# JackWoo0831/Yolov7-tracker

Measured on AMD Instinct MI355X. Metric: end-to-end fps (detect+track) YOLOv7-w6@1280 ByteTrack, higher is better.
Workload: dtype f16

## Files before the change

yolov7-tracker_amd/csrc/y7t_conv_ws_s2.hip:

```cpp
#include "y7t_common.h"
#include "y7t_conv_common.h"
#include <stdlib.h>

namespace {

#if defined(Y7T_CONVSIM)
#define WS2_VMCNT(dev, dma) cs_vmcnt(dma)
#else
#define WS2_VMCNT(dev, dma) asm volatile("s_waitcnt vmcnt(" #dev ")" ::: "memory")
#endif

struct Ws2 {
    static constexpr int TW = 32, TH = 2;
    static constexpr int PIXB = 144;
    static constexpr int NE = TW + 1, NO = TW;
    static constexpr int O_OFF = NE * PIXB;
    static constexpr int RP = (NE + NO) * PIXB;
    static constexpr int ROWS = 2 * TH + 1;
    static constexpr int PATCH_DMA = (ROWS * RP + 1023) / 1024;
    static constexpr int PATCH_BYTES = PATCH_DMA * 1024;
    static constexpr int NPW = (PATCH_DMA + 3) / 4;
    static constexpr int NBUF = 3;
    static constexpr int OUT_OFF = NBUF * PATCH_BYTES;
    static constexpr int LDS = OUT_OFF + TW * TH * 256;
    static constexpr int NSUB = 36;
    static constexpr unsigned OOB = 0xFF000000u;
};

template <int ACT, bool FUSE>
__global__ void __launch_bounds__(256, 1) k_conv3x3s2_c64_ws(const Y7TConvArgs p) {
#if defined(__HIP_DEVICE_COMPILE__)
    using C = Ws2;
    constexpr int TW = C::TW, TH = C::TH, PIXB = C::PIXB, RP = C::RP, NPW = C::NPW;
    extern __shared__ __attribute__((aligned(16))) char smem[];
    const int tid = threadIdx.x, lane = tid & 63, wave = __builtin_amdgcn_readfirstlane(tid >> 6);
    const int l31 = lane & 31, hi32 = lane >> 5;

    const int tiles_x = p.Wo / TW, tiles_y = p.Ho / TH, ptiles = p.B * tiles_y * tiles_x;
    int bid = blockIdx.x;
    if (p.xcd_swizzle) {
        const int nwg = gridDim.x, q = nwg >> 3, r = nwg & 7, xcd = bid & 7, idx = bid >> 3;
        bid = (xcd < r ? xcd * (q + 1) : r * (q + 1) + (xcd - r) * q) + idx;
    }
    const int per = (ptiles + (int)gridDim.x - 1) / (int)gridDim.x;
    const int pt_first = bid * per;
    const int nt = (ptiles - pt_first) < per ? (ptiles - pt_first) : per;
    if (nt <= 0) return;

    const __amdgpu_buffer_rsrc_t xr = __builtin_amdgcn_make_buffer_rsrc((void*)p.in, 0, p.in_bytes, 0x00020000);

    struct TileIt { int b, ty, tx, n; };
    auto tile_it = [&](int pt) -> TileIt {
        int q = pt;
        const int txi = q % tiles_x; q /= tiles_x;
        return TileIt{q / tiles_y, q % tiles_y, txi, pt_first + nt - pt};
    };
    auto tile_next = [&](TileIt& it) __attribute__((always_inline)) {
        it.n -= 1;
        if (++it.tx == tiles_x) { it.tx = 0; if (++it.ty == tiles_y) { it.ty = 0; ++it.b; } }
    };
    unsigned pconst[NPW], pedge = 0;
#pragma unroll
    for (int i = 0; i < NPW; ++i) {
        int I = wave + 4 * i;
        if (I >= C::PATCH_DMA) I = C::PATCH_DMA - 1;
        const int byte = I * 1024 + lane * 16;
        const int r = byte / RP, rb = byte - r * RP;
        const int px = rb / PIXB, cs = (rb - px * PIXB) >> 4;
        const int pc = px < C::NE ? 2 * px : 2 * (px - C::NE) + 1;
        const bool used = r < C::ROWS && cs < 8;
        pconst[i] = used ? (unsigned)(((r * p.W + pc) * p.ldin + cs * 8) * 2) : 0u;
        const unsigned e = used ? (unsigned)((r == 0) | ((pc == 0) << 1)) : 0u;
        pedge |= e << (2 * i);
    }
    auto piece_offsets = [&](const TileIt& it, unsigned (&pv)[NPW]) __attribute__((always_inline)) {
        const unsigned org = ((((unsigned)it.b * (unsigned)p.H + (unsigned)(2 * it.ty * TH) - 1u) * (unsigned)p.W + (unsigned)(2 * it.tx * TW) - 1u) * (unsigned)p.ldin +
                              (unsigned)p.cin_off) * 2u;
        const unsigned tmask = (unsigned)((it.ty == 0) | ((it.tx == 0) << 1));
#pragma unroll
        for (int i = 0; i < NPW; ++i) pv[i] = (it.n <= 0 || ((pedge >> (2 * i)) & tmask)) ? C::OOB : pconst[i] + org;
    };
    auto issue_piece = [&](int buf, unsigned v, int i) __attribute__((always_inline)) {
        const int I = (wave + 4 * i < C::PATCH_DMA) ? wave + 4 * i : C::PATCH_DMA - 1;
        __builtin_amdgcn_raw_ptr_buffer_load_lds(xr, (LDS_AS void*)(smem + buf * C::PATCH_BYTES + I * 1024), 16, v, 0, 0, 0);
    };

    half8 wreg[C::NSUB];
    {
        const half8* wp = (const half8*)p.w + wave * 64 + lane;
#pragma unroll
        for (int f = 0; f < C::NSUB; ++f) wreg[f] = wp[f * 256];
    }
    floatx16 biasv;
#pragma unroll
    for (int g = 0; g < 4; ++g)
#pragma unroll
        for (int e = 0; e < 4; ++e) biasv[g * 4 + e] = p.bias[wave * 32 + 8 * g + 4 * hi32 + e];

    half8 w2reg[FUSE ? 8 : 1];
    floatx16 bias2v;
    if (FUSE) {
        const half8* wp2 = (const half8*)p.w + C::NSUB * 256 + wave * 64 + lane;
#pragma unroll
        for (int ks = 0; ks < 8; ++ks) w2reg[ks] = wp2[ks * 256];
#pragma unroll
        for (int g = 0; g < 4; ++g)
#pragma unroll
            for (int e = 0; e < 4; ++e) bias2v[g * 4 + e] = p.bias[128 + wave * 32 + 8 * g + 4 * hi32 + e];
    }

    unsigned pv[NPW];
    TileIt itn = tile_it(pt_first), ito = itn;
    piece_offsets(itn, pv);
#pragma unroll
    for (int i = 0; i < NPW; ++i) issue_piece(0, pv[i], i);
    tile_next(itn);
    piece_offsets(itn, pv);
#pragma unroll
    for (int i = 0; i < NPW; ++i) issue_piece(1, pv[i], i);
    tile_next(itn);

    const int plane_off = l31 * PIXB + hi32 * 16;
    half_t* outp = (half_t*)p.out;
    typedef __attribute__((ext_vector_type(4))) unsigned uint4v;

    char* og = smem + C::OUT_OFF;
    auto put_chunk = [&](const float* y, int c) __attribute__((always_inline)) {
        const int j = c >> 1, gp = c & 1, pix = j * 32 + l31;
        typedef __attribute__((ext_vector_type(2))) _Float16 half2v;
        unsigned w[2][2];
#pragma unroll
        for (int gg = 0; gg < 2; ++gg) {
            half2v h0 = {(half_t)y[gg * 4 + 0], (half_t)y[gg * 4 + 1]}, h1 = {(half_t)y[gg * 4 + 2], (half_t)y[gg * 4 + 3]};
            w[gg][0] = __builtin_bit_cast(unsigned, h0);
            w[gg][1] = __builtin_bit_cast(unsigned, h1);
        }
        auto r0 = __builtin_amdgcn_permlane32_swap(w[0][0], w[1][0], false, false);
        auto r1 = __builtin_amdgcn_permlane32_swap(w[0][1], w[1][1], false, false);
        const uint4v pk = {r0[0], r1[0], r0[1], r1[1]};
        const int ch = wave * 4 + gp * 2 + hi32;
        *(uint4v*)(og + pix * 256 + ((ch ^ (pix & 15)) << 4)) = pk;
    };
    auto gather = [&](const floatx16 (&a)[2]) __attribute__((always_inline)) {
#pragma unroll
        for (int c = 0; c < 4; ++c) {
            float y[8];
#pragma unroll
            for (int e = 0; e < 8; ++e) y[e] = act_t<ACT>(a[c >> 1][(c & 1) * 8 + e]);
            put_chunk(y, c);
        }
    };
    auto store_tile = [&](const TileIt& it) __attribute__((always_inline)) {
        const int oy = it.ty * TH, ox = it.tx * TW;
        uint4v v[4];
#pragma unroll
        for (int k = 0; k < 4; ++k) {
            const int c = k * 256 + tid, pix = c >> 4, ch = c & 15;
            v[k] = *(const uint4v*)(og + pix * 256 + ((ch ^ (pix & 15)) << 4));
        }
        __builtin_amdgcn_sched_barrier(0);
#pragma unroll
        for (int k = 0; k < 4; ++k) {
            const int c = k * 256 + tid, pix = c >> 4, ch = c & 15;
            const int gy = oy + (pix >> 5), gx = ox + (pix & 31);
            *(uint4v*)(outp + ((size_t)(it.b * p.Ho + gy) * p.Wo + gx) * p.ldout + p.cout_off + ch * 8) = v[k];
        }
    };
    floatx16 acc2[2];

    int buf = 0;
    for (int t = 0; t < nt; ++t) {
        const int nbuf = (buf + 2 >= C::NBUF) ? buf + 2 - C::NBUF : buf + 2;
        static_assert(NPW == 12, "the waits below count the pieces and stores of a tile");
        if (t == 0) WS2_VMCNT(12, 12);
        else if (t == 1) WS2_VMCNT(16, 12);
        else WS2_VMCNT(20, 12);
        __builtin_amdgcn_s_barrier();
        piece_offsets(itn, pv);
#pragma unroll
        for (int i = 0; i < NPW; ++i) issue_piece(nbuf, pv[i], i);
        tile_next(itn);

        const char* pb = smem + buf * C::PATCH_BYTES + plane_off;
        floatx16 acc[2];
        auto frag = [&](int sn, int j) __attribute__((always_inline)) -> half8 {
            const int tap = sn >> 2, ks = sn & 3, kh = tap / 3, kw = tap - kh * 3;
            return *(const half8*)(pb + (2 * j + kh) * RP + (kw == 1 ? C::O_OFF : kw == 2 ? PIXB : 0) + ks * 32);
        };
        half8 xq[3][2];
#pragma unroll
        for (int q = 0; q < 3; ++q)
#pragma unroll
            for (int j = 0; j < 2; ++j) xq[q][j] = frag(q, j);
        __builtin_amdgcn_sched_barrier(0);
#pragma unroll
        for (int s = 0; s < C::NSUB; ++s) {
#pragma unroll
            for (int j = 0; j < 2; ++j) {
                acc[j] = __builtin_amdgcn_mfma_f32_32x32x16_f16(wreg[s], xq[s % 3][j], s == 0 ? biasv : acc[j], 0, 0, 0);
                if (s + 3 < C::NSUB) xq[s % 3][j] = frag(s + 3, j);
                __builtin_amdgcn_sched_barrier(0);
            }
        }
        gather(acc);
        if (FUSE) {
            __builtin_amdgcn_s_barrier();
            auto frag2 = [&](int ks, int j) __attribute__((always_inline)) -> half8 {
                const int pix = j * 32 + l31, ch = ks * 2 + hi32;
                return *(const half8*)(og + pix * 256 + ((ch ^ (pix & 15)) << 4));
            };
            half8 x2[3][2];
#pragma unroll
            for (int q = 0; q < 3; ++q)
#pragma unroll
                for (int j = 0; j < 2; ++j) x2[q][j] = frag2(q, j);
            __builtin_amdgcn_sched_barrier(0);
#pragma unroll
            for (int ks = 0; ks < 8; ++ks)
#pragma unroll
                for (int j = 0; j < 2; ++j) {
                    acc2[j] = __builtin_amdgcn_mfma_f32_32x32x16_f16(w2reg[ks], x2[ks % 3][j], ks == 0 ? bias2v : acc2[j], 0, 0, 0);
                    if (ks + 3 < 8) x2[ks % 3][j] = frag2(ks + 3, j);
                    __builtin_amdgcn_sched_barrier(0);
                }
            __builtin_amdgcn_s_barrier();
            gather(acc2);
        }
        __builtin_amdgcn_s_barrier();
        store_tile(ito);
        tile_next(ito);
        buf = (buf + 1 == C::NBUF) ? 0 : buf + 1;
    }
    WS2_VMCNT(0, 0);
#endif
}

}

int y7t_conv_ws_s2_launch(const Y7TConvArgs& a, hipStream_t s) {
    using C = Ws2;
    const bool ok = a.KH == 3 && a.KW == 3 && a.stride == 2 && a.pad == 1 && a.Cin == 64 && a.Cout == 128 && a.Cout_pad == 128 && !a.out_f32 && !(a.ldout & 7) &&
                    !(a.cout_off & 7) && !(a.ldin & 7) && !(a.cin_off & 7) && !(a.H & 1) && !(a.W & 1) && a.Ho * 2 == a.H && a.Wo * 2 == a.W && a.in_bytes < 0x80000000u &&
                    a.Ho % C::TH == 0 && a.Wo % C::TW == 0 && !a.epi && a.up_C == 0;
    if (!ok) {
        y7t_set_error("conv: weights are in the stride-2 register-fragment order (korder 8) but the layer is not a 3x3 / stride 2 / 64 -> 128 convolution of an even map "
                      "whose output is whole 2 x 32 tiles with an aligned fp16 output");
        return Y7T_E_ARG;
    }
    static Y7TOncePerDevice attr;
    if (int e_ = y7t_once_per_device(attr, [&]() -> int {
#define WS2_ATTR(ACT) Y7T_HIP_CHECK(hipFuncSetAttribute((const void*)k_conv3x3s2_c64_ws<ACT, false>, hipFuncAttributeMaxDynamicSharedMemorySize, C::LDS)); \
                      Y7T_HIP_CHECK(hipFuncSetAttribute((const void*)k_conv3x3s2_c64_ws<ACT, true>, hipFuncAttributeMaxDynamicSharedMemorySize, C::LDS));
        WS2_ATTR(Y7T_ACT_NONE) WS2_ATTR(Y7T_ACT_SILU) WS2_ATTR(Y7T_ACT_LEAKY)
#undef WS2_ATTR
        return 0;
    })) return e_;
    static int wgs_env = -2;
    if (wgs_env == -2) wgs_env = y7t_exp_switch("Y7T_CONV_WS_WGS", -1);
    const int ncu = wgs_env > 0 ? wgs_env : y7t_num_cus();
    const int ptiles = a.B * (a.Ho / C::TH) * (a.Wo / C::TW);
    const int grid = ptiles < ncu ? ptiles : ncu;
    const bool fuse = a.korder == 11;
#define WS2_GO(ACT) do { if (fuse) hipLaunchKernelGGL((k_conv3x3s2_c64_ws<ACT, true>), dim3(grid), dim3(256), C::LDS, s, a); \
                         else hipLaunchKernelGGL((k_conv3x3s2_c64_ws<ACT, false>), dim3(grid), dim3(256), C::LDS, s, a); } while (0)
    if (a.act == Y7T_ACT_SILU) WS2_GO(Y7T_ACT_SILU);
    else if (a.act == Y7T_ACT_LEAKY) WS2_GO(Y7T_ACT_LEAKY);
    else WS2_GO(Y7T_ACT_NONE);
#undef WS2_GO
    Y7T_LAUNCH_CHECK();
    y7t_note_kernel(fuse ? "ws_s2<2,32> + 1x1" : "ws_s2<2,32>");
    return 0;
}
```

yolov7-tracker_amd/csrc/y7t_stem.hip:

```cpp
#include "y7t_common.h"
#include "y7t_conv_common.h"
#include <stdlib.h>

namespace {

constexpr int TS = 16;
constexpr int PS = TS + 2;
constexpr int PIXB = 48;
constexpr int PATCH_BYTES = PS * PS * PIXB;

struct StemArgs {
    const uint8_t* img;
    int B, H0, W0;
    int H, W;
    int new_h, new_w, top, left;
    const _Float16* w;
    int K_pad;
    const float* bias;
    _Float16* out;
    int ldout, cout_off, act;
    int tiles_x, tiles_y, n_tiles;
};

template <bool RESIZE>
__device__ __forceinline__ void lb_pixel(const StemArgs& p, int b, int y, int x, float sy, float sx, float* bgr) {
    const int yy = y - p.top, xx = x - p.left;
    bgr[0] = bgr[1] = bgr[2] = 114.f;
    if ((unsigned)yy >= (unsigned)p.new_h || (unsigned)xx >= (unsigned)p.new_w) return;
    if (!RESIZE) {
        const uint8_t* s = p.img + (((size_t)b * p.H0 + yy) * p.W0 + xx) * 3;
        bgr[0] = s[0]; bgr[1] = s[1]; bgr[2] = s[2];
        return;
    }
    const float fy = ((float)yy + 0.5f) * sy - 0.5f, fx = ((float)xx + 0.5f) * sx - 0.5f;
    int y0 = (int)floorf(fy), x0 = (int)floorf(fx);
    const float wy = fy - (float)y0, wx = fx - (float)x0;
    const int y1 = min(max(y0 + 1, 0), p.H0 - 1), x1 = min(max(x0 + 1, 0), p.W0 - 1);
    y0 = min(max(y0, 0), p.H0 - 1); x0 = min(max(x0, 0), p.W0 - 1);
    const uint8_t* r0 = p.img + ((size_t)b * p.H0 + y0) * p.W0 * 3;
    const uint8_t* r1 = p.img + ((size_t)b * p.H0 + y1) * p.W0 * 3;
    for (int c = 0; c < 3; ++c) {
        const float t0 = (1.f - wx) * r0[x0 * 3 + c] + wx * r0[x1 * 3 + c];
        const float t1 = (1.f - wx) * r1[x0 * 3 + c] + wx * r1[x1 * 3 + c];
        bgr[c] = rintf((1.f - wy) * t0 + wy * t1);
    }
}

template <bool RESIZE, bool LINES>
__global__ void __launch_bounds__(256, 2) k_stem_u8(const StemArgs p) {
#if defined(__HIP_DEVICE_COMPILE__)
    extern __shared__ __attribute__((aligned(16))) char smem[];
    const int tid = threadIdx.x, lane = tid & 63, wave = tid >> 6;
    const int l31 = lane & 31, hi32 = lane >> 5;
    const int Hr = p.H >> 1, Wr = p.W >> 1;
    const float sy = (float)p.H0 / (float)p.new_h, sx = (float)p.W0 / (float)p.new_w;

    half8 wf[9][2];
#pragma unroll
    for (int t = 0; t < 9; ++t)
#pragma unroll
        for (int i = 0; i < 2; ++i) wf[t][i] = *(const half8*)(p.w + (size_t)(i * 32 + l31) * p.K_pad + t * 16 + hi32 * 8);
    float bv[2][4][4];
#pragma unroll
    for (int i = 0; i < 2; ++i)
#pragma unroll
        for (int g = 0; g < 4; ++g)
#pragma unroll
            for (int e = 0; e < 4; ++e) bv[i][g][e] = p.bias[i * 32 + 8 * g + 4 * hi32 + e];

    auto fetch_raw = [&](int tile, int q, unsigned short (&raw)[2][3], int& flags) {
        flags = 0;
        int tt = tile < p.n_tiles ? tile : 0;
        const int txi = tt % p.tiles_x; tt /= p.tiles_x;
        const int tyi = tt % p.tiles_y, b = tt / p.tiles_y;
        const int qq = q < PS * PS ? q : 0;
        const int ry = qq / PS, rx = qq - ry * PS;
        const int gy = tyi * TS - 1 + ry, gx = txi * TS - 1 + rx;
        if (q < PS * PS && tile < p.n_tiles && (unsigned)gy < (unsigned)Hr && (unsigned)gx < (unsigned)Wr) flags |= 1;
        const int xx = 2 * gx - p.left;
        if ((unsigned)xx < (unsigned)p.new_w) flags |= 8;
        const int xc = min(max(xx, 0), p.W0 - 2);
#pragma unroll
        for (int dy = 0; dy < 2; ++dy) {
            const int yy = 2 * gy + dy - p.top;
            if ((unsigned)yy < (unsigned)p.new_h) flags |= 2 << dy;
            const int yc = min(max(yy, 0), p.H0 - 1);
            const unsigned short* sp = (const unsigned short*)(p.img + (((size_t)b * p.H0 + yc) * p.W0 + xc) * 3);
            raw[dy][0] = sp[0]; raw[dy][1] = sp[1]; raw[dy][2] = sp[2];
        }
    };
    auto convert_raw = [&](const unsigned short (&raw)[2][3], int flags, half_t* v) {
#pragma unroll
        for (int c = 12; c < 16; ++c) v[c] = (half_t)0.f;
#pragma unroll
        for (int dy = 0; dy < 2; ++dy) {
            const bool ok = (flags & 8) && (flags & (2 << dy));
            const unsigned w0 = raw[dy][0] | ((unsigned)raw[dy][1] << 16), w1 = raw[dy][2];
            const unsigned char by[6] = {(unsigned char)w0, (unsigned char)(w0 >> 8), (unsigned char)(w0 >> 16), (unsigned char)(w0 >> 24),
                                         (unsigned char)w1, (unsigned char)(w1 >> 8)};
#pragma unroll
            for (int dx = 0; dx < 2; ++dx)
#pragma unroll
                for (int ch = 0; ch < 3; ++ch) {
                    const float u = ok ? (float)by[dx * 3 + (2 - ch)] : 114.f;
                    v[(dy + 2 * dx) * 3 + ch] = (flags & 1) ? (half_t)(u * 0.00392156862745098f) : (half_t)0.f;
                }
        }
    };
    auto fetch = [&](int tile, int q, half_t* v) {
#pragma unroll
        for (int c = 0; c < 16; ++c) v[c] = (half_t)0.f;
        if (q >= PS * PS || tile >= p.n_tiles) return;
        int tt = tile;
        const int txi = tt % p.tiles_x; tt /= p.tiles_x;
        const int tyi = tt % p.tiles_y, b = tt / p.tiles_y;
        const int ry = q / PS, rx = q - ry * PS;
        const int gy = tyi * TS - 1 + ry, gx = txi * TS - 1 + rx;
        if ((unsigned)gy >= (unsigned)Hr || (unsigned)gx >= (unsigned)Wr) return;
#pragma unroll
        for (int g = 0; g < 4; ++g) {
            float bgr[3];
            lb_pixel<true>(p, b, 2 * gy + (g & 1), 2 * gx + (g >> 1), sy, sx, bgr);
#pragma unroll
            for (int ch = 0; ch < 3; ++ch) v[g * 3 + ch] = (half_t)(bgr[2 - ch] / 255.0f);
        }
    };
    auto store_patch = [&](char* patch, int q, const half_t* v) {
        if (q >= PS * PS) return;
        *(half8*)(patch + q * PIXB) = *(const half8*)v;
        *(half8*)(patch + q * PIXB + 16) = *(const half8*)(v + 8);
    };
    unsigned short ra[2][3], rb[2][3];
    int fa = 0, fb = 0;
    auto fetch_pair = [&](int tile, half_t* va_, half_t* vb_) {
        if (RESIZE) { fetch(tile, tid, va_); fetch(tile, tid + 256, vb_); }
        else { fetch_raw(tile, tid, ra, fa); fetch_raw(tile, tid + 256, rb, fb); }
    };
    auto finish_pair = [&](half_t* va_, half_t* vb_) {
        if (!RESIZE) { convert_raw(ra, fa, va_); convert_raw(rb, fb, vb_); }
    };

    const int t0 = blockIdx.x;
    half_t va[16], vb[16];
    fetch_pair(t0, va, vb);
    finish_pair(va, vb);
    store_patch(smem, tid, va); store_patch(smem, tid + 256, vb);
    __syncthreads();
    int cur = 0;
    for (int tile = t0; tile < p.n_tiles; tile += gridDim.x) {
        const int nxt = tile + gridDim.x;
        fetch_pair(nxt, va, vb);
        const char* patch = smem + cur * PATCH_BYTES;
        floatx16 acc[2][2];
#pragma unroll
        for (int i = 0; i < 2; ++i)
#pragma unroll
            for (int j = 0; j < 2; ++j)
#pragma unroll
                for (int e = 0; e < 16; ++e) acc[i][j][e] = 0.f;
#pragma unroll
        for (int t = 0; t < 9; ++t) {
            const int kh = t / 3, kw = t - kh * 3;
            half8 xf[2];
#pragma unroll
            for (int j = 0; j < 2; ++j) {
                const int row = (wave * 2 + j) * 2 + (l31 >> 4), x = l31 & 15;
                xf[j] = *(const half8*)(patch + ((row + kh) * PS + x + kw) * PIXB + hi32 * 16);
            }
#pragma unroll
            for (int i = 0; i < 2; ++i)
#pragma unroll
                for (int j = 0; j < 2; ++j) acc[i][j] = __builtin_amdgcn_mfma_f32_32x32x16_f16(wf[t][i], xf[j], acc[i][j], 0, 0, 0);
        }
        int tt = tile;
        const int txi = tt % p.tiles_x; tt /= p.tiles_x;
        const int tyi = tt % p.tiles_y, b = tt / p.tiles_y;
        act_dispatch(p.act, [&](auto act_c) {
            constexpr int ACT = decltype(act_c)::value;
#pragma unroll
            for (int j = 0; j < 2; ++j) {
                const int gy = tyi * TS + (wave * 2 + j) * 2 + (l31 >> 4), gx = txi * TS + (l31 & 15);
                const bool okp = gy < Hr && gx < Wr;
                half_t* orow = p.out + ((size_t)(b * Hr + gy) * Wr + gx) * p.ldout + p.cout_off;
                char* scr = smem + 2 * PATCH_BYTES + wave * 4096;
#pragma unroll
                for (int i = 0; i < 2; ++i)
#pragma unroll
                    for (int gp = 0; gp < 2; ++gp) {
                        unsigned w[2][2];
#pragma unroll
                        for (int gg = 0; gg < 2; ++gg) {
                            const int g = gp * 2 + gg;
                            float v[4];
#pragma unroll
                            for (int e = 0; e < 4; ++e) v[e] = act_t<ACT>(acc[i][j][g * 4 + e] + bv[i][g][e]);
                            typedef __attribute__((ext_vector_type(2))) _Float16 half2v;
                            half2v h0v = {(half_t)v[0], (half_t)v[1]}, h1v = {(half_t)v[2], (half_t)v[3]};
                            w[gg][0] = __builtin_bit_cast(unsigned, h0v);
                            w[gg][1] = __builtin_bit_cast(unsigned, h1v);
                        }
                        auto r0 = __builtin_amdgcn_permlane32_swap(w[0][0], w[1][0], false, false);
                        auto r1 = __builtin_amdgcn_permlane32_swap(w[0][1], w[1][1], false, false);
                        typedef __attribute__((ext_vector_type(4))) unsigned uint4v;
                        const uint4v pk = {r0[0], r1[0], r0[1], r1[1]};
                        const int nn = i * 32 + 8 * (gp * 2 + hi32);
                        if (LINES) *(uint4v*)(scr + l31 * 128 + (((nn >> 3) ^ (l31 & 7)) << 4)) = pk;
                        else if (okp) *(uint4v*)(orow + nn) = pk;
                    }
                if (LINES) {
                    typedef __attribute__((ext_vector_type(4))) unsigned uint4v;
#pragma unroll
                    for (int k = 0; k < 4; ++k) {
                        const int px = k * 8 + (lane >> 3), ch = lane & 7;
                        const uint4v v4 = *(const uint4v*)(scr + px * 128 + ((ch ^ (px & 7)) << 4));
                        const int py = tyi * TS + (wave * 2 + j) * 2 + (px >> 4), pxx = txi * TS + (px & 15);
                        if (py < Hr && pxx < Wr) *(uint4v*)(p.out + ((size_t)(b * Hr + py) * Wr + pxx) * p.ldout + p.cout_off + ch * 8) = v4;
                    }
                }
            }
        });
        char* np_ = smem + (cur ^ 1) * PATCH_BYTES;
        finish_pair(va, vb);
        store_patch(np_, tid, va); store_patch(np_, tid + 256, vb);
        __syncthreads();
        cur ^= 1;
    }
#endif
}

}

int y7t_stem_u8_launch(const void* frames_u8, int B, int H0, int W0, int H, int W, int new_h, int new_w, int top, int left, const _Float16* w, int K_pad,
                       const float* bias, _Float16* out, int ldout, int cout_off, int act, hipStream_t s) {
    if ((H & 31) || (W & 31) || ldout % 8 || cout_off % 8) { y7t_set_error("stem: image %dx%d / output slice not supported", H, W); return Y7T_E_ARG; }
    StemArgs a;
    a.img = (const uint8_t*)frames_u8; a.B = B; a.H0 = H0; a.W0 = W0; a.H = H; a.W = W; a.new_h = new_h; a.new_w = new_w; a.top = top; a.left = left;
    a.w = w; a.K_pad = K_pad; a.bias = bias; a.out = out; a.ldout = ldout; a.cout_off = cout_off; a.act = act;
    a.tiles_x = (W / 2 + TS - 1) / TS; a.tiles_y = (H / 2 + TS - 1) / TS; a.n_tiles = B * a.tiles_x * a.tiles_y;
    const bool resize = !(new_h == H0 && new_w == W0 && (left & 1) == 0 && (W0 & 1) == 0 && W0 >= 2);
    int grid = a.n_tiles < 2048 ? a.n_tiles : 2048;
    static Y7TOncePerDevice attr;
    constexpr int LDSL = 2 * PATCH_BYTES + 4 * 4096;
    if (int e_ = y7t_once_per_device(attr, [&]() -> int {
        Y7T_HIP_CHECK(hipFuncSetAttribute((const void*)k_stem_u8<true, false>, hipFuncAttributeMaxDynamicSharedMemorySize, 2 * PATCH_BYTES));
        Y7T_HIP_CHECK(hipFuncSetAttribute((const void*)k_stem_u8<false, false>, hipFuncAttributeMaxDynamicSharedMemorySize, 2 * PATCH_BYTES));
        Y7T_HIP_CHECK(hipFuncSetAttribute((const void*)k_stem_u8<false, true>, hipFuncAttributeMaxDynamicSharedMemorySize, LDSL));
        return 0;
    })) return e_;
    static const int lines = y7t_exp_switch("Y7T_STEM_LINES", 1);
    if (resize) hipLaunchKernelGGL((k_stem_u8<true, false>), dim3(grid), dim3(256), 2 * PATCH_BYTES, s, a);
    else if (lines) hipLaunchKernelGGL((k_stem_u8<false, true>), dim3(grid), dim3(256), LDSL, s, a);
    else hipLaunchKernelGGL((k_stem_u8<false, false>), dim3(grid), dim3(256), 2 * PATCH_BYTES, s, a);
    Y7T_LAUNCH_CHECK();
    y7t_note_kernel("stem_u8<%s>", resize ? "letterbox-resize" : "direct");
    return 0;
}
```

Baseline: 2467.

## Streamline stem kernel addressing and add ablation switches to stride-2 conv

The stem kernel now advances tile coordinates incrementally instead of recomputing them with divisions, precomputes per-thread patch and output offsets in 32-bit arithmetic, and makes the activation a template parameter instead of dispatching at run time. The raw-pixel conversion becomes branch-free through masking. A guard rejects launches over 2 GiB so the 32-bit offsets stay valid. The stride-2 conv gains compile-time ablation variants that are reachable only under a build flag and environment switch, so they are experiment scaffolding.

```diff
diff --git a/yolov7-tracker_amd/csrc/y7t_conv_ws_s2.hip b/yolov7-tracker_amd/csrc/y7t_conv_ws_s2.hip
--- a/yolov7-tracker_amd/csrc/y7t_conv_ws_s2.hip
+++ b/yolov7-tracker_amd/csrc/y7t_conv_ws_s2.hip
@@ -6,7 +6,9 @@
 
 #if defined(Y7T_CONVSIM)
 #define WS2_VMCNT(dev, dma) cs_vmcnt(dma)
+#define WS2_KEEP(a) (void)(a)
 #else
+#define WS2_KEEP(a) asm volatile("" ::"v"((a)[0]), "v"((a)[1]))
 #define WS2_VMCNT(dev, dma) asm volatile("s_waitcnt vmcnt(" #dev ")" ::: "memory")
 #endif
 
@@ -27,7 +29,7 @@
     static constexpr unsigned OOB = 0xFF000000u;
 };
 
-template <int ACT, bool FUSE>
+template <int ACT, bool FUSE, int ABL = 0>
 __global__ void __launch_bounds__(256, 1) k_conv3x3s2_c64_ws(const Y7TConvArgs p) {
 #if defined(__HIP_DEVICE_COMPILE__)
     using C = Ws2;
@@ -146,7 +148,7 @@
         for (int c = 0; c < 4; ++c) {
             float y[8];
 #pragma unroll
-            for (int e = 0; e < 8; ++e) y[e] = act_t<ACT>(a[c >> 1][(c & 1) * 8 + e]);
+            for (int e = 0; e < 8; ++e) y[e] = (ABL & 32) ? a[c >> 1][(c & 1) * 8 + e] : act_t<ACT>(a[c >> 1][(c & 1) * 8 + e]);
             put_chunk(y, c);
         }
     };
@@ -172,13 +174,14 @@
     for (int t = 0; t < nt; ++t) {
         const int nbuf = (buf + 2 >= C::NBUF) ? buf + 2 - C::NBUF : buf + 2;
         static_assert(NPW == 12, "the waits below count the pieces and stores of a tile");
-        if (t == 0) WS2_VMCNT(12, 12);
+        if (ABL & 8) {}
+        else if (t == 0) WS2_VMCNT(12, 12);
         else if (t == 1) WS2_VMCNT(16, 12);
         else WS2_VMCNT(20, 12);
-        __builtin_amdgcn_s_barrier();
+        if (!(ABL & 8)) __builtin_amdgcn_s_barrier();
         piece_offsets(itn, pv);
 #pragma unroll
-        for (int i = 0; i < NPW; ++i) issue_piece(nbuf, pv[i], i);
+        for (int i = 0; i < NPW; ++i) if (!(ABL & 2)) issue_piece(nbuf, pv[i], i);
         tile_next(itn);
 
         const char* pb = smem + buf * C::PATCH_BYTES + plane_off;
@@ -202,9 +205,9 @@
                 __builtin_amdgcn_sched_barrier(0);
             }
         }
-        gather(acc);
+        if (ABL & 1) { WS2_KEEP(acc); } else gather(acc);
         if (FUSE) {
-            __builtin_amdgcn_s_barrier();
+            if (!(ABL & 8)) __builtin_amdgcn_s_barrier();
             auto frag2 = [&](int ks, int j) __attribute__((always_inline)) -> half8 {
                 const int pix = j * 32 + l31, ch = ks * 2 + hi32;
                 return *(const half8*)(og + pix * 256 + ((ch ^ (pix & 15)) << 4));
@@ -223,11 +226,11 @@
                     if (ks + 3 < 8) x2[ks % 3][j] = frag2(ks + 3, j);
                     __builtin_amdgcn_sched_barrier(0);
                 }
-            __builtin_amdgcn_s_barrier();
-            gather(acc2);
-        }
-        __builtin_amdgcn_s_barrier();
-        store_tile(ito);
+            if (!(ABL & 8)) __builtin_amdgcn_s_barrier();
+            if (ABL & 1) { WS2_KEEP(acc2); } else gather(acc2);
+        }
+        if (!(ABL & 8)) __builtin_amdgcn_s_barrier();
+        if (!(ABL & 16)) store_tile(ito);
         tile_next(ito);
         buf = (buf + 1 == C::NBUF) ? 0 : buf + 1;
     }
@@ -261,6 +264,25 @@
     const int ptiles = a.B * (a.Ho / C::TH) * (a.Wo / C::TW);
     const int grid = ptiles < ncu ? ptiles : ncu;
     const bool fuse = a.korder == 11;
+#if Y7T_ABLATE
+    static int abl = -1;
+    if (abl < 0) abl = y7t_exp_switch("Y7T_WS2_ABLATE", 0);
+    if (abl && fuse && a.act == Y7T_ACT_SILU) {
+#define Y7T_WS2_ABL_CASE(N) \
+        case N: \
+            Y7T_HIP_CHECK(hipFuncSetAttribute((const void*)k_conv3x3s2_c64_ws<Y7T_ACT_SILU, true, N>, hipFuncAttributeMaxDynamicSharedMemorySize, C::LDS)); \
+            hipLaunchKernelGGL((k_conv3x3s2_c64_ws<Y7T_ACT_SILU, true, N>), dim3(grid), dim3(256), C::LDS, s, a); \
+            break;
+        switch (abl) {
+            Y7T_WS2_ABL_CASE(1) Y7T_WS2_ABL_CASE(2) Y7T_WS2_ABL_CASE(8) Y7T_WS2_ABL_CASE(16) Y7T_WS2_ABL_CASE(17) Y7T_WS2_ABL_CASE(32) Y7T_WS2_ABL_CASE(27)
+            default: y7t_set_error("conv: unknown Y7T_WS2_ABLATE value"); return Y7T_E_ARG;
+        }
+#undef Y7T_WS2_ABL_CASE
+        Y7T_LAUNCH_CHECK();
+        y7t_note_kernel("ws_s2<2,32> + 1x1");
+        return 0;
+    }
+#endif
 #define WS2_GO(ACT) do { if (fuse) hipLaunchKernelGGL((k_conv3x3s2_c64_ws<ACT, true>), dim3(grid), dim3(256), C::LDS, s, a); \
                          else hipLaunchKernelGGL((k_conv3x3s2_c64_ws<ACT, false>), dim3(grid), dim3(256), C::LDS, s, a); } while (0)
     if (a.act == Y7T_ACT_SILU) WS2_GO(Y7T_ACT_SILU);
diff --git a/yolov7-tracker_amd/csrc/y7t_stem.hip b/yolov7-tracker_amd/csrc/y7t_stem.hip
--- a/yolov7-tracker_amd/csrc/y7t_stem.hip
+++ b/yolov7-tracker_amd/csrc/y7t_stem.hip
@@ -46,11 +46,11 @@
     }
 }
 
-template <bool RESIZE, bool LINES>
+template <bool RESIZE, bool LINES, int ACT>
 __global__ void __launch_bounds__(256, 2) k_stem_u8(const StemArgs p) {
 #if defined(__HIP_DEVICE_COMPILE__)
     extern __shared__ __attribute__((aligned(16))) char smem[];
-    const int tid = threadIdx.x, lane = tid & 63, wave = tid >> 6;
+    const int tid = threadIdx.x, lane = tid & 63, wave = __builtin_amdgcn_readfirstlane(tid >> 6);
     const int l31 = lane & 31, hi32 = lane >> 5;
     const int Hr = p.H >> 1, Wr = p.W >> 1;
     const float sy = (float)p.H0 / (float)p.new_h, sx = (float)p.W0 / (float)p.new_w;
@@ -68,89 +68,132 @@
 #pragma unroll
             for (int e = 0; e < 4; ++e) bv[i][g][e] = p.bias[i * 32 + 8 * g + 4 * hi32 + e];
 
-    auto fetch_raw = [&](int tile, int q, unsigned short (&raw)[2][3], int& flags) {
+    struct TileIt { int n, b, ty, tx; };
+    const int gsz = (int)gridDim.x;
+    const int sdx = gsz % p.tiles_x, sdy = (gsz / p.tiles_x) % p.tiles_y, sdb = (gsz / p.tiles_x) / p.tiles_y;
+    auto tile_step = [&](TileIt& it) __attribute__((always_inline)) {
+        it.n += gsz;
+        it.tx += sdx;
+        int c = it.tx >= p.tiles_x;
+        it.tx -= c ? p.tiles_x : 0;
+        it.ty += sdy + c;
+        c = it.ty >= p.tiles_y;
+        it.ty -= c ? p.tiles_y : 0;
+        it.b += sdb + c;
+    };
+
+    int pry[2], prx[2];
+    bool pq[2];
+#pragma unroll
+    for (int h = 0; h < 2; ++h) {
+        const int q = tid + 256 * h;
+        pq[h] = q < PS * PS;
+        const int qq = pq[h] ? q : 0;
+        pry[h] = qq / PS; prx[h] = qq - pry[h] * PS;
+    }
+    const unsigned W3 = (unsigned)p.W0 * 3u;
+    auto fetch_raw = [&](const TileIt& it, int h, unsigned short (&raw)[2][3], int& flags) __attribute__((always_inline)) {
         flags = 0;
-        int tt = tile < p.n_tiles ? tile : 0;
-        const int txi = tt % p.tiles_x; tt /= p.tiles_x;
-        const int tyi = tt % p.tiles_y, b = tt / p.tiles_y;
-        const int qq = q < PS * PS ? q : 0;
-        const int ry = qq / PS, rx = qq - ry * PS;
-        const int gy = tyi * TS - 1 + ry, gx = txi * TS - 1 + rx;
-        if (q < PS * PS && tile < p.n_tiles && (unsigned)gy < (unsigned)Hr && (unsigned)gx < (unsigned)Wr) flags |= 1;
+        const bool live = it.n < p.n_tiles;
+        const int b = live ? it.b : 0, tyi = live ? it.ty : 0, txi = live ? it.tx : 0;
+        const int gy = tyi * TS - 1 + pry[h], gx = txi * TS - 1 + prx[h];
+        if (pq[h] && live && (unsigned)gy < (unsigned)Hr && (unsigned)gx < (unsigned)Wr) flags |= 1;
         const int xx = 2 * gx - p.left;
         if ((unsigned)xx < (unsigned)p.new_w) flags |= 8;
         const int xc = min(max(xx, 0), p.W0 - 2);
+        const unsigned rowb = (unsigned)(b * p.H0);
 #pragma unroll
         for (int dy = 0; dy < 2; ++dy) {
             const int yy = 2 * gy + dy - p.top;
             if ((unsigned)yy < (unsigned)p.new_h) flags |= 2 << dy;
             const int yc = min(max(yy, 0), p.H0 - 1);
-            const unsigned short* sp = (const unsigned short*)(p.img + (((size_t)b * p.H0 + yc) * p.W0 + xc) * 3);
+            const unsigned short* sp = (const unsigned short*)(p.img + ((rowb + (unsigned)yc) * W3 + (unsigned)xc * 3u));
             raw[dy][0] = sp[0]; raw[dy][1] = sp[1]; raw[dy][2] = sp[2];
         }
     };
-    auto convert_raw = [&](const unsigned short (&raw)[2][3], int flags, half_t* v) {
+    auto convert_raw = [&](const unsigned short (&raw)[2][3], int flags, half_t* v) __attribute__((always_inline)) {
+        typedef __attribute__((ext_vector_type(2))) _Float16 half2v;
 #pragma unroll
         for (int c = 12; c < 16; ++c) v[c] = (half_t)0.f;
 #pragma unroll
         for (int dy = 0; dy < 2; ++dy) {
             const bool ok = (flags & 8) && (flags & (2 << dy));
-            const unsigned w0 = raw[dy][0] | ((unsigned)raw[dy][1] << 16), w1 = raw[dy][2];
+            const unsigned w0 = ok ? raw[dy][0] | ((unsigned)raw[dy][1] << 16) : 0x72727272u, w1 = ok ? (unsigned)raw[dy][2] : 0x7272u;
             const unsigned char by[6] = {(unsigned char)w0, (unsigned char)(w0 >> 8), (unsigned char)(w0 >> 16), (unsigned char)(w0 >> 24),
                                          (unsigned char)w1, (unsigned char)(w1 >> 8)};
 #pragma unroll
             for (int dx = 0; dx < 2; ++dx)
 #pragma unroll
                 for (int ch = 0; ch < 3; ++ch) {
-                    const float u = ok ? (float)by[dx * 3 + (2 - ch)] : 114.f;
-                    v[(dy + 2 * dx) * 3 + ch] = (flags & 1) ? (half_t)(u * 0.00392156862745098f) : (half_t)0.f;
+                    const float u = (float)by[dx * 3 + (2 - ch)];
+                    v[(dy + 2 * dx) * 3 + ch] = (half_t)(u * 0.00392156862745098f);
                 }
         }
-    };
-    auto fetch = [&](int tile, int q, half_t* v) {
+        const unsigned inside = (flags & 1) ? 0xFFFFFFFFu : 0u;
+#pragma unroll
+        for (int k = 0; k < 6; ++k) {
+            half2v h = {v[2 * k], v[2 * k + 1]};
+            h = __builtin_bit_cast(half2v, __builtin_bit_cast(unsigned, h) & inside);
+            v[2 * k] = h[0]; v[2 * k + 1] = h[1];
+        }
+    };
+    auto fetch = [&](const TileIt& it, int h, half_t* v) {
 #pragma unroll
         for (int c = 0; c < 16; ++c) v[c] = (half_t)0.f;
-        if (q >= PS * PS || tile >= p.n_tiles) return;
-        int tt = tile;
-        const int txi = tt % p.tiles_x; tt /= p.tiles_x;
-        const int tyi = tt % p.tiles_y, b = tt / p.tiles_y;
-        const int ry = q / PS, rx = q - ry * PS;
-        const int gy = tyi * TS - 1 + ry, gx = txi * TS - 1 + rx;
+        if (!pq[h] || it.n >= p.n_tiles) return;
+        const int gy = it.ty * TS - 1 + pry[h], gx = it.tx * TS - 1 + prx[h];
         if ((unsigned)gy >= (unsigned)Hr || (unsigned)gx >= (unsigned)Wr) return;
 #pragma unroll
         for (int g = 0; g < 4; ++g) {
             float bgr[3];
-            lb_pixel<true>(p, b, 2 * gy + (g & 1), 2 * gx + (g >> 1), sy, sx, bgr);
+            lb_pixel<true>(p, it.b, 2 * gy + (g & 1), 2 * gx + (g >> 1), sy, sx, bgr);
 #pragma unroll
             for (int ch = 0; ch < 3; ++ch) v[g * 3 + ch] = (half_t)(bgr[2 - ch] / 255.0f);
         }
     };
-    auto store_patch = [&](char* patch, int q, const half_t* v) {
-        if (q >= PS * PS) return;
+    auto store_patch = [&](char* patch, int h, const half_t* v) __attribute__((always_inline)) {
+        if (!pq[h]) return;
+        const int q = tid + 256 * h;
         *(half8*)(patch + q * PIXB) = *(const half8*)v;
         *(half8*)(patch + q * PIXB + 16) = *(const half8*)(v + 8);
     };
     unsigned short ra[2][3], rb[2][3];
     int fa = 0, fb = 0;
-    auto fetch_pair = [&](int tile, half_t* va_, half_t* vb_) {
-        if (RESIZE) { fetch(tile, tid, va_); fetch(tile, tid + 256, vb_); }
-        else { fetch_raw(tile, tid, ra, fa); fetch_raw(tile, tid + 256, rb, fb); }
-    };
-    auto finish_pair = [&](half_t* va_, half_t* vb_) {
+    auto fetch_pair = [&](const TileIt& it, half_t* va_, half_t* vb_) __attribute__((always_inline)) {
+        if (RESIZE) { fetch(it, 0, va_); fetch(it, 1, vb_); }
+        else { fetch_raw(it, 0, ra, fa); fetch_raw(it, 1, rb, fb); }
+    };
+    auto finish_pair = [&](half_t* va_, half_t* vb_) __attribute__((always_inline)) {
         if (!RESIZE) { convert_raw(ra, fa, va_); convert_raw(rb, fb, vb_); }
     };
 
-    const int t0 = blockIdx.x;
+    const int fragoff = ((wave * 4 + (l31 >> 4)) * PS + (l31 & 15)) * PIXB + hi32 * 16;
+    const unsigned ldo = (unsigned)p.ldout;
+    const unsigned oreg = ((unsigned)((wave * 4 + (l31 >> 4)) * Wr + (l31 & 15)) * ldo + 8u * hi32) * 2u;
+    const unsigned oline = ((unsigned)((wave * 4) * Wr + (lane >> 3)) * ldo + 8u * (lane & 7)) * 2u;
+    const unsigned jstep = 2u * (unsigned)Wr * ldo * 2u;
+    char* const scr = smem + 2 * PATCH_BYTES + wave * 4096;
+    const int scr_w = l31 * 128, scr_r = (lane >> 3) * 128 + (((lane & 7) ^ ((lane >> 3) & 7)) << 4);
+    typedef __attribute__((ext_vector_type(4))) unsigned uint4v;
+
+    TileIt cur_t;
+    {
+        int tt = (int)blockIdx.x;
+        cur_t.n = tt;
+        cur_t.tx = tt % p.tiles_x; tt /= p.tiles_x;
+        cur_t.ty = tt % p.tiles_y; cur_t.b = tt / p.tiles_y;
+    }
+    TileIt nxt_t = cur_t;
     half_t va[16], vb[16];
-    fetch_pair(t0, va, vb);
+    fetch_pair(cur_t, va, vb);
     finish_pair(va, vb);
-    store_patch(smem, tid, va); store_patch(smem, tid + 256, vb);
+    store_patch(smem, 0, va); store_patch(smem, 1, vb);
     __syncthreads();
     int cur = 0;
-    for (int tile = t0; tile < p.n_tiles; tile += gridDim.x) {
-        const int nxt = tile + gridDim.x;
-        fetch_pair(nxt, va, vb);
-        const char* patch = smem + cur * PATCH_BYTES;
+    for (; cur_t.n < p.n_tiles; cur_t = nxt_t) {
+        tile_step(nxt_t);
+        fetch_pair(nxt_t, va, vb);
+        const char* patch = smem + cur * PATCH_BYTES + fragoff;
         floatx16 acc[2][2];
 #pragma unroll
         for (int i = 0; i < 2; ++i)
@@ -163,65 +206,50 @@
             const int kh = t / 3, kw = t - kh * 3;
             half8 xf[2];
 #pragma unroll
-            for (int j = 0; j < 2; ++j) {
-                const int row = (wave * 2 + j) * 2 + (l31 >> 4), x = l31 & 15;
-                xf[j] = *(const half8*)(patch + ((row + kh) * PS + x + kw) * PIXB + hi32 * 16);
-            }
+            for (int j = 0; j < 2; ++j) xf[j] = *(const half8*)(patch + ((2 * j + kh) * PS + kw) * PIXB);
 #pragma unroll
             for (int i = 0; i < 2; ++i)
 #pragma unroll
                 for (int j = 0; j < 2; ++j) acc[i][j] = __builtin_amdgcn_mfma_f32_32x32x16_f16(wf[t][i], xf[j], acc[i][j], 0, 0, 0);
         }
-        int tt = tile;
-        const int txi = tt % p.tiles_x; tt /= p.tiles_x;
-        const int tyi = tt % p.tiles_y, b = tt / p.tiles_y;
-        act_dispatch(p.act, [&](auto act_c) {
-            constexpr int ACT = decltype(act_c)::value;
-#pragma unroll
-            for (int j = 0; j < 2; ++j) {
-                const int gy = tyi * TS + (wave * 2 + j) * 2 + (l31 >> 4), gx = txi * TS + (l31 & 15);
-                const bool okp = gy < Hr && gx < Wr;
-                half_t* orow = p.out + ((size_t)(b * Hr + gy) * Wr + gx) * p.ldout + p.cout_off;
-                char* scr = smem + 2 * PATCH_BYTES + wave * 4096;
-#pragma unroll
-                for (int i = 0; i < 2; ++i)
-#pragma unroll
-                    for (int gp = 0; gp < 2; ++gp) {
-                        unsigned w[2][2];
-#pragma unroll
-                        for (int gg = 0; gg < 2; ++gg) {
-                            const int g = gp * 2 + gg;
-                            float v[4];
-#pragma unroll
-                            for (int e = 0; e < 4; ++e) v[e] = act_t<ACT>(acc[i][j][g * 4 + e] + bv[i][g][e]);
-                            typedef __attribute__((ext_vector_type(2))) _Float16 half2v;
-                            half2v h0v = {(half_t)v[0], (half_t)v[1]}, h1v = {(half_t)v[2], (half_t)v[3]};
-                            w[gg][0] = __builtin_bit_cast(unsigned, h0v);
-                            w[gg][1] = __builtin_bit_cast(unsigned, h1v);
-                        }
-                        auto r0 = __builtin_amdgcn_permlane32_swap(w[0][0], w[1][0], false, false);
-                        auto r1 = __builtin_amdgcn_permlane32_swap(w[0][1], w[1][1], false, false);
-                        typedef __attribute__((ext_vector_type(4))) unsigned uint4v;
-                        const uint4v pk = {r0[0], r1[0], r0[1], r1[1]};
-                        const int nn = i * 32 + 8 * (gp * 2 + hi32);
-                        if (LINES) *(uint4v*)(scr + l31 * 128 + (((nn >> 3) ^ (l31 & 7)) << 4)) = pk;
-                        else if (okp) *(uint4v*)(orow + nn) = pk;
+        const unsigned tbase = ((unsigned)((cur_t.b * Hr + cur_t.ty * TS) * Wr + cur_t.tx * TS) * ldo + (unsigned)p.cout_off) * 2u;
+        char* const ob = (char*)p.out + tbase;
+#pragma unroll
+        for (int j = 0; j < 2; ++j) {
+#pragma unroll
+            for (int i = 0; i < 2; ++i)
+#pragma unroll
+                for (int gp = 0; gp < 2; ++gp) {
+                    unsigned w[2][2];
+#pragma unroll
+                    for (int gg = 0; gg < 2; ++gg) {
+                        const int g = gp * 2 + gg;
+                        float v[4];
+#pragma unroll
+                        for (int e = 0; e < 4; ++e) v[e] = act_t<ACT>(acc[i][j][g * 4 + e] + bv[i][g][e]);
+                        typedef __attribute__((ext_vector_type(2))) _Float16 half2v;
+                        half2v h0v = {(half_t)v[0], (half_t)v[1]}, h1v = {(half_t)v[2], (half_t)v[3]};
+                        w[gg][0] = __builtin_bit_cast(unsigned, h0v);
+                        w[gg][1] = __builtin_bit_cast(unsigned, h1v);
                     }
-                if (LINES) {
-                    typedef __attribute__((ext_vector_type(4))) unsigned uint4v;
-#pragma unroll
-                    for (int k = 0; k < 4; ++k) {
-                        const int px = k * 8 + (lane >> 3), ch = lane & 7;
-                        const uint4v v4 = *(const uint4v*)(scr + px * 128 + ((ch ^ (px & 7)) << 4));
-                        const int py = tyi * TS + (wave * 2 + j) * 2 + (px >> 4), pxx = txi * TS + (px & 15);
-                        if (py < Hr && pxx < Wr) *(uint4v*)(p.out + ((size_t)(b * Hr + py) * Wr + pxx) * p.ldout + p.cout_off + ch * 8) = v4;
-                    }
+                    auto r0 = __builtin_amdgcn_permlane32_swap(w[0][0], w[1][0], false, false);
+                    auto r1 = __builtin_amdgcn_permlane32_swap(w[0][1], w[1][1], false, false);
+                    const uint4v pk = {r0[0], r1[0], r0[1], r1[1]};
+                    const int cn = i * 4 + gp * 2;
+                    if (LINES) *(uint4v*)(scr + scr_w + (((cn + hi32) ^ (l31 & 7)) << 4)) = pk;
+                    else *(uint4v*)(ob + (j * jstep + oreg + cn * 16)) = pk;
+                }
+            if (LINES) {
+#pragma unroll
+                for (int k = 0; k < 4; ++k) {
+                    const uint4v v4 = *(const uint4v*)(scr + k * 1024 + scr_r);
+                    *(uint4v*)(ob + (j * jstep + ((unsigned)((k >> 1) * Wr + (k & 1) * 8) * ldo) * 2u + oline)) = v4;
                 }
             }
-        });
+        }
         char* np_ = smem + (cur ^ 1) * PATCH_BYTES;
         finish_pair(va, vb);
-        store_patch(np_, tid, va); store_patch(np_, tid + 256, vb);
+        store_patch(np_, 0, va); store_patch(np_, 1, vb);
         __syncthreads();
         cur ^= 1;
     }
@@ -239,18 +267,30 @@
     a.tiles_x = (W / 2 + TS - 1) / TS; a.tiles_y = (H / 2 + TS - 1) / TS; a.n_tiles = B * a.tiles_x * a.tiles_y;
     const bool resize = !(new_h == H0 && new_w == W0 && (left & 1) == 0 && (W0 & 1) == 0 && W0 >= 2);
     int grid = a.n_tiles < 2048 ? a.n_tiles : 2048;
+    if ((long long)B * H0 * W0 * 3 >= (1ll << 31) || (long long)B * (H / 2) * (W / 2) * ldout * 2 >= (1ll << 31)) {
+        y7t_set_error("stem: the frames or the output of one launch pass 2 GiB");
+        return Y7T_E_ARG;
+    }
     static Y7TOncePerDevice attr;
     constexpr int LDSL = 2 * PATCH_BYTES + 4 * 4096;
     if (int e_ = y7t_once_per_device(attr, [&]() -> int {
-        Y7T_HIP_CHECK(hipFuncSetAttribute((const void*)k_stem_u8<true, false>, hipFuncAttributeMaxDynamicSharedMemorySize, 2 * PATCH_BYTES));
-        Y7T_HIP_CHECK(hipFuncSetAttribute((const void*)k_stem_u8<false, false>, hipFuncAttributeMaxDynamicSharedMemorySize, 2 * PATCH_BYTES));
-        Y7T_HIP_CHECK(hipFuncSetAttribute((const void*)k_stem_u8<false, true>, hipFuncAttributeMaxDynamicSharedMemorySize, LDSL));
+#define STEM_ATTR(ACT) \
+        Y7T_HIP_CHECK(hipFuncSetAttribute((const void*)k_stem_u8<true, false, ACT>, hipFuncAttributeMaxDynamicSharedMemorySize, 2 * PATCH_BYTES)); \
+        Y7T_HIP_CHECK(hipFuncSetAttribute((const void*)k_stem_u8<false, false, ACT>, hipFuncAttributeMaxDynamicSharedMemorySize, 2 * PATCH_BYTES)); \
+        Y7T_HIP_CHECK(hipFuncSetAttribute((const void*)k_stem_u8<false, true, ACT>, hipFuncAttributeMaxDynamicSharedMemorySize, LDSL));
+        STEM_ATTR(Y7T_ACT_NONE) STEM_ATTR(Y7T_ACT_SILU) STEM_ATTR(Y7T_ACT_LEAKY)
+#undef STEM_ATTR
         return 0;
     })) return e_;
     static const int lines = y7t_exp_switch("Y7T_STEM_LINES", 1);
-    if (resize) hipLaunchKernelGGL((k_stem_u8<true, false>), dim3(grid), dim3(256), 2 * PATCH_BYTES, s, a);
-    else if (lines) hipLaunchKernelGGL((k_stem_u8<false, true>), dim3(grid), dim3(256), LDSL, s, a);
-    else hipLaunchKernelGGL((k_stem_u8<false, false>), dim3(grid), dim3(256), 2 * PATCH_BYTES, s, a);
+#define STEM_GO(ACT) do { \
+        if (resize) hipLaunchKernelGGL((k_stem_u8<true, false, ACT>), dim3(grid), dim3(256), 2 * PATCH_BYTES, s, a); \
+        else if (lines) hipLaunchKernelGGL((k_stem_u8<false, true, ACT>), dim3(grid), dim3(256), LDSL, s, a); \
+        else hipLaunchKernelGGL((k_stem_u8<false, false, ACT>), dim3(grid), dim3(256), 2 * PATCH_BYTES, s, a); } while (0)
+    if (act == Y7T_ACT_SILU) STEM_GO(Y7T_ACT_SILU);
+    else if (act == Y7T_ACT_LEAKY) STEM_GO(Y7T_ACT_LEAKY);
+    else STEM_GO(Y7T_ACT_NONE);
+#undef STEM_GO
     Y7T_LAUNCH_CHECK();
     y7t_note_kernel("stem_u8<%s>", resize ? "letterbox-resize" : "direct");
     return 0;
```

After: 2476, median of 6. About the same (+0.4%).
